# Acmece/rl-collision-avoidance

Hardware: AMD Instinct MI355X
Metric: agent-steps/s (N robots x 512-beam lidar) (higher is better)
Workload: dtype f32

## Files before the change

rl-collision-avoidance_amd/csrc/mrca_abi.hip:

```cpp
#include <hip/hip_runtime.h>
#include <string>
#include <chrono>

#include <algorithm>
#include <cmath>
#include <cstdarg>
#include <cstdio>
#include <cstdlib>
#include <cstring>
#include <memory>
#include <mutex>
#include <new>
#include <type_traits>
#include <utility>
#include <vector>

#include "../../include/mrca_env.h"
#include "mrca_host.h"
#include "mrca_hostutil.h"
#include "mrca_kernels.h"
#include "mrca_orca.h"
#include "mrca_dwa.h"
#include "mrca_pass_plan.h"
#include "mrca_render.h"
#include "mrca_rollout_store.h"

namespace {
thread_local char g_err[512] = "";
}

namespace mrca {
int set_error(int code, const char* fmt, ...) {
    va_list ap;
    va_start(ap, fmt);
    vsnprintf(g_err, sizeof(g_err), fmt, ap);
    va_end(ap);
    return code;
}
}

namespace {

using mrca::DeviceGuard;
using mrca::kAheadTicks;
#define fail(...) mrca::set_error(__VA_ARGS__)

#define HIP_TRY(expr)                                                                               \
    do {                                                                                            \
        hipError_t _e = (expr);                                                                     \
        if (_e != hipSuccess) return fail(MRCA_ERR_HIP, "%s failed: %s", #expr, hipGetErrorString(_e)); \
    } while (0)

constexpr size_t kAlign = 256;
size_t align_up(size_t v) { return (v + kAlign - 1) / kAlign * kAlign; }

struct Layout {
    size_t field_off[MRCA_F_COUNT];
    size_t field_bytes[MRCA_F_COUNT];
    size_t off_reset_mode, off_goal_mode, off_group_id, off_init_table, off_goal_table;
    size_t off_beam_cos, off_beam_sin, off_map, off_free_rect, off_cellfield, off_head, off_outline;
    size_t off_bw_ticket, off_bw_prov, off_bw_state, off_bw_chead, off_bw_cnext, off_bw_lstart, off_bw_lcount, off_bw_lsorted, off_bw_lblock, off_bw_lcursor;
    size_t off_status;
    int32_t bw_cmask, bw_lmask;
    size_t total;
};

int validate(const mrca_config* c) {
    if (!c) return fail(MRCA_ERR_INVALID, "config is NULL");
    if (c->abi_version != MRCA_ABI_VERSION)
        return fail(MRCA_ERR_INVALID, "abi_version %d != %d", c->abi_version, MRCA_ABI_VERSION);
    if (c->num_worlds < 1) return fail(MRCA_ERR_INVALID, "num_worlds must be >= 1");
    if (c->robots_per_world < 1) return fail(MRCA_ERR_INVALID, "robots_per_world must be >= 1");
    if (c->robots_per_world > 64 && c->auto_reset == MRCA_AUTO_GROUP)
        return fail(MRCA_ERR_UNSUPPORTED, "robots_per_world %d > 64 with group-synchronous episodes (auto_reset 2)",
                    c->robots_per_world);
    if (!(c->collision_raster >= 0.0f)) return fail(MRCA_ERR_INVALID, "collision_raster must be >= 0");
    if (c->collision_raster > 0.0f && (c->collision_raster < 0.1f || mrca::outline_span(1.0f / c->collision_raster) > mrca::kOutlineWin))
        return fail(MRCA_ERR_UNSUPPORTED, "collision_raster %.3f m: an outline is kept as an 8 x 8 bitmap of raster cells, which "
                    "holds cells of >= 0.1 m", (double)c->collision_raster);
    if (c->collision_raster > 0.0f && c->robots_per_world > 64)
        return fail(MRCA_ERR_UNSUPPORTED, "collision_raster with robots_per_world > 64");
    if ((int64_t)c->num_worlds * c->robots_per_world > (1 << 24))
        return fail(MRCA_ERR_UNSUPPORTED, "more than 2^24 robots in one environment");
    if (c->beams < 64 || c->beams > 1024 || c->beams % 64)
        return fail(MRCA_ERR_INVALID, "beams %d must be a multiple of 64 in [64,1024]", c->beams);
    if (c->frames < 1 || c->frames > 8) return fail(MRCA_ERR_INVALID, "frames %d out of [1,8]", c->frames);
    if (c->map_width < 1 || c->map_height < 1 || c->map_words_per_row < (c->map_width + 31) / 32)
        return fail(MRCA_ERR_INVALID, "bad map geometry %dx%d wpr %d", c->map_width, c->map_height,
                    c->map_words_per_row);
    if (c->map_width > 16384 || c->map_height > 16384)
        return fail(MRCA_ERR_UNSUPPORTED, "map %dx%d cells: at most 16384 per side", c->map_width, c->map_height);
    if (!(c->map_cell > 0.0f)) return fail(MRCA_ERR_INVALID, "map_cell must be > 0");
    if (!c->map_bits) return fail(MRCA_ERR_INVALID, "map_bits is NULL");
    if (c->auto_reset < 0 || c->auto_reset > 2) return fail(MRCA_ERR_INVALID, "auto_reset %d", c->auto_reset);
    const int R = c->robots_per_world;
    for (int i = 0; i < R; ++i) {
        if (c->reset_mode && (c->reset_mode[i] < 0 || c->reset_mode[i] > 2))
            return fail(MRCA_ERR_INVALID, "reset_mode[%d] = %d", i, c->reset_mode[i]);
        if (c->goal_mode && (c->goal_mode[i] < 0 || c->goal_mode[i] > 2))
            return fail(MRCA_ERR_INVALID, "goal_mode[%d] = %d", i, c->goal_mode[i]);
        if (c->group_id && (c->group_id[i] < 0 || c->group_id[i] > 15))
            return fail(MRCA_ERR_INVALID, "group_id[%d] = %d out of [0,15]", i, c->group_id[i]);
        if (c->reset_mode && c->reset_mode[i] == MRCA_RESET_TABLE && !c->init_table)
            return fail(MRCA_ERR_INVALID, "reset_mode[%d] is TABLE but init_table is NULL", i);
        if (c->goal_mode && c->goal_mode[i] == MRCA_RESET_TABLE && !c->goal_table)
            return fail(MRCA_ERR_INVALID, "goal_mode[%d] is TABLE but goal_table is NULL", i);
    }
    return MRCA_OK;
}

void make_layout(const mrca_config* c, Layout* L) {
    const size_t N = (size_t)c->num_worlds * c->robots_per_world;
    const size_t B = c->beams, F = c->frames, R = c->robots_per_world;
    size_t sz[MRCA_F_COUNT];
    sz[MRCA_F_POSE] = N * 3 * 4;
    sz[MRCA_F_SPEED] = N * 2 * 4;
    sz[MRCA_F_SPEED_GT] = N * 2 * 4;
    sz[MRCA_F_GOAL] = N * 2 * 4;
    sz[MRCA_F_INIT_POSE] = N * 3 * 4;
    sz[MRCA_F_SCAN] = N * B * 4;
    sz[MRCA_F_OBS] = N * F * B * 4;
    sz[MRCA_F_LOCAL_GOAL] = N * 2 * 4;
    sz[MRCA_F_REWARD] = N * 4;
    sz[MRCA_F_DONE] = N;
    sz[MRCA_F_RESULT] = N;
    sz[MRCA_F_FIRST_RESULT] = N;
    sz[MRCA_F_CRASHED] = N;
    sz[MRCA_F_LIVE] = N;
    sz[MRCA_F_FRESH] = N;
    sz[MRCA_F_T] = N * 4;
    sz[MRCA_F_EPISODE] = N * 4;
    sz[MRCA_F_PREV_DIST] = N * 4;
    sz[MRCA_F_SCAN_RING] = N * F * B * 4;
    sz[MRCA_F_RING_HEAD] = N;
    sz[MRCA_F_HIT_BITS] = N * F * (B / 64) * 8;
    size_t off = 0;
    for (int f = 0; f < MRCA_F_COUNT; ++f) {
        L->field_off[f] = off;
        L->field_bytes[f] = sz[f];
        off += align_up(sz[f]);
    }
    auto take = [&](size_t bytes) {
        size_t o = off;
        off += align_up(bytes);
        return o;
    };
    L->off_reset_mode = take(R * 4);
    L->off_goal_mode = take(R * 4);
    L->off_group_id = take(R * 4);
    L->off_init_table = take(R * 3 * 4);
    L->off_goal_table = take(R * 2 * 4);
    L->off_beam_cos = take(B * 4);
    L->off_beam_sin = take(B * 4);
    L->off_map = take((size_t)c->map_height * c->map_words_per_row * 4);
    L->off_free_rect = take((size_t)(c->map_width + 2 * mrca::kFieldPadX) * (c->map_height + 2 * mrca::kFieldPadY) *
                            4 * sizeof(uint16_t));
    L->off_cellfield = take((size_t)c->map_width * c->map_height);
    L->off_head = take(N * sizeof(float4));
    L->off_outline = take(c->collision_raster > 0.0f ? N * sizeof(mrca::OutlineBits) : 0);
    L->bw_cmask = L->bw_lmask = 0;
    if (c->robots_per_world > 64) {
        size_t mc = 1, ml = 1;
        while (mc < 4 * N) mc <<= 1;
        while (ml < 2 * N) ml <<= 1;
        L->bw_cmask = (int32_t)(mc - 1);
        L->bw_lmask = (int32_t)(ml - 1);
        L->off_bw_ticket = take(4);
        L->off_bw_prov = take(N * 2 * sizeof(float4));
        L->off_bw_state = take(N * 4);
        L->off_bw_chead = take(mc * 4);
        L->off_bw_cnext = take(2 * N * 4);
        L->off_bw_lstart = take((ml + 2) * 4);
        L->off_bw_lcount = take((ml + 1) * 4);
        L->off_bw_lsorted = take(N * 4);
// ... 196 lines not shown
    env->view.dev = env->view_dev.get();
    if ((e = hipDeviceSynchronize()) != hipSuccess) return e;
    return hipMemcpy(env->view_dev.get(), &env->view, sizeof(mrca::EnvView), hipMemcpyHostToDevice);
}

static int attach_arena(mrca_env* env, void* arena_dev, size_t arena_bytes) {
    const size_t total = env->layout.total;
    if (arena_dev) {
        if (arena_bytes < total) return fail(MRCA_ERR_NOMEM, "arena of %zu bytes < required %zu", arena_bytes, total);
        if (reinterpret_cast<uintptr_t>(arena_dev) % kAlign) return fail(MRCA_ERR_INVALID, "arena must be %zu-byte aligned", kAlign);
        env->arena = static_cast<char*>(arena_dev);
        return MRCA_OK;
    }
    const hipError_t e = device_alloc(&env->own_arena, total);
    if (e != hipSuccess) return fail(MRCA_ERR_NOMEM, "hipMalloc(%zu) failed: %s", total, hipGetErrorString(e));
    env->arena = env->own_arena.get();
    return MRCA_OK;
}

static int upload_tables(const mrca_config* cfg, const Layout& L, char* arena, int* free_rect_pitch, int* num_groups_out) {
    HIP_TRY(hipMemset(arena, 0, L.total));
    const int R = cfg->robots_per_world, B = cfg->beams;
    const size_t N = (size_t)cfg->num_worlds * R;
    std::vector<int32_t> reset_mode(R, MRCA_RESET_DISC), goal_mode(R, MRCA_RESET_DISC), group(R, 0);
    std::vector<float> init_tab(R * 3, 0.0f), goal_tab(R * 2, 0.0f);
    if (cfg->reset_mode) memcpy(reset_mode.data(), cfg->reset_mode, R * 4);
    if (cfg->goal_mode) memcpy(goal_mode.data(), cfg->goal_mode, R * 4);
    else if (cfg->reset_mode) goal_mode = reset_mode;
    if (cfg->group_id) memcpy(group.data(), cfg->group_id, R * 4);
    if (cfg->init_table) memcpy(init_tab.data(), cfg->init_table, R * 3 * 4);
    if (cfg->goal_table) memcpy(goal_tab.data(), cfg->goal_table, R * 2 * 4);
    int num_groups = 0;
    for (int i = 0; i < R; ++i) num_groups = group[i] + 1 > num_groups ? group[i] + 1 : num_groups;
    *num_groups_out = num_groups;
    std::vector<float> bcos(B), bsin(B);
    for (int i = 0; i < B; ++i) {
        const double b = -M_PI / 2.0 + (double)i * (M_PI / (double)(B - 1));
        bcos[i] = (float)std::cos(b);
        bsin[i] = (float)std::sin(b);
    }
    HIP_TRY(hipMemcpy(arena + L.off_reset_mode, reset_mode.data(), R * 4, hipMemcpyHostToDevice));
    HIP_TRY(hipMemcpy(arena + L.off_goal_mode, goal_mode.data(), R * 4, hipMemcpyHostToDevice));
    HIP_TRY(hipMemcpy(arena + L.off_group_id, group.data(), R * 4, hipMemcpyHostToDevice));
    HIP_TRY(hipMemcpy(arena + L.off_init_table, init_tab.data(), R * 3 * 4, hipMemcpyHostToDevice));
    HIP_TRY(hipMemcpy(arena + L.off_goal_table, goal_tab.data(), R * 2 * 4, hipMemcpyHostToDevice));
    {
        std::vector<float> pose0((size_t)N * 3);
        for (size_t n = 0; n < N; ++n)
            for (int k = 0; k < 3; ++k) pose0[n * 3 + k] = init_tab[(n % (size_t)R) * 3 + k];
        HIP_TRY(hipMemcpy(arena + L.field_off[MRCA_F_POSE], pose0.data(), pose0.size() * 4, hipMemcpyHostToDevice));
    }
    HIP_TRY(hipMemcpy(arena + L.off_beam_cos, bcos.data(), B * 4, hipMemcpyHostToDevice));
    HIP_TRY(hipMemcpy(arena + L.off_beam_sin, bsin.data(), B * 4, hipMemcpyHostToDevice));
    HIP_TRY(hipMemcpy(arena + L.off_map, cfg->map_bits, (size_t)cfg->map_height * cfg->map_words_per_row * 4,
                      hipMemcpyHostToDevice));
    {
        const std::shared_ptr<const HostField> hf = host_field(cfg, false);
        *free_rect_pitch = hf->pitch;
        HIP_TRY(hipMemcpy(arena + L.off_free_rect, hf->entries.data(), hf->entries.size() * sizeof(uint16_t),
                          hipMemcpyHostToDevice));
    }
    {
        std::vector<uint8_t> cf;
        mrca::build_cell_field(cfg->map_bits, cfg->map_width, cfg->map_height, cfg->map_words_per_row, &cf);
        HIP_TRY(hipMemcpy(arena + L.off_cellfield, cf.data(), cf.size(), hipMemcpyHostToDevice));
    }
    if (R > 64)
        HIP_TRY(hipMemset(arena + L.off_bw_chead, 0xFF, ((size_t)L.bw_cmask + 1) * 4));
    HIP_TRY(hipMemset(arena + L.field_off[MRCA_F_LIVE], 1, N));
    {
        std::vector<int32_t> ones(N, 1);
        HIP_TRY(hipMemcpy(arena + L.field_off[MRCA_F_T], ones.data(), N * 4, hipMemcpyHostToDevice));
    }
    return MRCA_OK;
}

static bool field_octants(const mrca_config* c) {
    if (const char* v = std::getenv("MRCA_FIELD_OCTANTS")) return std::atoi(v) != 0;
    const size_t bytes = (size_t)(c->map_width + 2 * mrca::kFieldPadX) * (c->map_height + 2 * mrca::kFieldPadY) * 8 * sizeof(uint16_t);
    return c->lazy_obs != 0 && bytes <= ((size_t)4 << 20);
}

static int upload_octants(const mrca_config* cfg, mrca_env* env) {
    const std::shared_ptr<const HostField> hf = host_field(cfg, true);
    const size_t bytes = hf->octants.size() * sizeof(uint16_t);
    HIP_TRY(device_alloc(&env->octant_rect, bytes));
    HIP_TRY(hipMemcpy(env->octant_rect.get(), hf->octants.data(), bytes, hipMemcpyHostToDevice));
    env->view.march_rect = env->octant_rect.get();
    env->view.march_shift = 4;
    env->view.march_major = 8;
    return MRCA_OK;
}

static mrca::EnvView make_view(const mrca_config* cfg, const Layout& L, char* a, int free_rect_pitch, int num_groups) {
    const int R = cfg->robots_per_world, B = cfg->beams;
    const size_t N = (size_t)cfg->num_worlds * R;
    mrca::EnvView v = mrca::EnvView();
    v.N = (int32_t)N;
    v.R = R;
    v.W = cfg->num_worlds;
    v.B = B;
    v.F = cfg->frames;
    v.pose = reinterpret_cast<float*>(a + L.field_off[MRCA_F_POSE]);
    v.speed = reinterpret_cast<float*>(a + L.field_off[MRCA_F_SPEED]);
    v.speed_gt = reinterpret_cast<float*>(a + L.field_off[MRCA_F_SPEED_GT]);
    v.goal = reinterpret_cast<float*>(a + L.field_off[MRCA_F_GOAL]);
    v.init_pose = reinterpret_cast<float*>(a + L.field_off[MRCA_F_INIT_POSE]);
    v.scan = reinterpret_cast<float*>(a + L.field_off[MRCA_F_SCAN]);
    v.obs = reinterpret_cast<float*>(a + L.field_off[MRCA_F_OBS]);
    v.scan_ring = reinterpret_cast<float*>(a + L.field_off[MRCA_F_SCAN_RING]);
    v.ring_head = reinterpret_cast<uint8_t*>(a + L.field_off[MRCA_F_RING_HEAD]);
    v.hit_bits = reinterpret_cast<unsigned long long*>(a + L.field_off[MRCA_F_HIT_BITS]);
    v.local_goal = reinterpret_cast<float*>(a + L.field_off[MRCA_F_LOCAL_GOAL]);
    v.reward = reinterpret_cast<float*>(a + L.field_off[MRCA_F_REWARD]);
    v.prev_dist = reinterpret_cast<float*>(a + L.field_off[MRCA_F_PREV_DIST]);
    v.done = reinterpret_cast<uint8_t*>(a + L.field_off[MRCA_F_DONE]);
    v.result = reinterpret_cast<uint8_t*>(a + L.field_off[MRCA_F_RESULT]);
    v.first_result = reinterpret_cast<uint8_t*>(a + L.field_off[MRCA_F_FIRST_RESULT]);
    v.crashed = reinterpret_cast<uint8_t*>(a + L.field_off[MRCA_F_CRASHED]);
    v.live = reinterpret_cast<uint8_t*>(a + L.field_off[MRCA_F_LIVE]);
    v.fresh = reinterpret_cast<uint8_t*>(a + L.field_off[MRCA_F_FRESH]);
    v.t = reinterpret_cast<int32_t*>(a + L.field_off[MRCA_F_T]);
    v.episode = reinterpret_cast<int32_t*>(a + L.field_off[MRCA_F_EPISODE]);
    v.reset_mode = reinterpret_cast<const int32_t*>(a + L.off_reset_mode);
    v.goal_mode = reinterpret_cast<const int32_t*>(a + L.off_goal_mode);
    v.group_id = reinterpret_cast<const int32_t*>(a + L.off_group_id);
    v.init_table = reinterpret_cast<const float*>(a + L.off_init_table);
    v.goal_table = reinterpret_cast<const float*>(a + L.off_goal_table);
    v.beam_cos = reinterpret_cast<const float*>(a + L.off_beam_cos);
    v.beam_sin = reinterpret_cast<const float*>(a + L.off_beam_sin);
    v.beam_step = mrca::kPi / (float)(B - 1);
    v.beam_inv_step = (float)(B - 1) / mrca::kPi;
    v.map_bits = reinterpret_cast<const uint32_t*>(a + L.off_map);
    v.free_rect = reinterpret_cast<const uint16_t*>(a + L.off_free_rect);
    v.free_rect_pitch = free_rect_pitch;
    v.march_rect = v.free_rect;
    v.march_shift = 3;
    v.march_major = 0;
    v.cellfield = reinterpret_cast<const uint8_t*>(a + L.off_cellfield);
    v.head = reinterpret_cast<float4*>(a + L.off_head);
    v.outline = cfg->collision_raster > 0.0f ? reinterpret_cast<mrca::OutlineBits*>(a + L.off_outline) : nullptr;
    v.big = R > 64 ? 1 : 0;
    if (v.big) {
        v.bw_ticket = reinterpret_cast<uint32_t*>(a + L.off_bw_ticket);
        v.bw_prov = reinterpret_cast<float4*>(a + L.off_bw_prov);
        v.bw_state = reinterpret_cast<int32_t*>(a + L.off_bw_state);
        v.bw_chead = reinterpret_cast<int32_t*>(a + L.off_bw_chead);
        v.bw_cnext = reinterpret_cast<int32_t*>(a + L.off_bw_cnext);
        v.bw_lstart = reinterpret_cast<int32_t*>(a + L.off_bw_lstart);
        v.bw_lcount = reinterpret_cast<int32_t*>(a + L.off_bw_lcount);
        v.bw_lsorted = reinterpret_cast<int32_t*>(a + L.off_bw_lsorted);
        v.bw_lblock = reinterpret_cast<int32_t*>(a + L.off_bw_lblock);
        v.bw_lcursor = reinterpret_cast<int32_t*>(a + L.off_bw_lcursor);
        v.bw_cmask = L.bw_cmask;
        v.bw_lmask = L.bw_lmask;
    }
    v.status = reinterpret_cast<uint32_t*>(a + L.off_status);
    v.ray_first = 0;
    v.ray_count = (int32_t)N;
    v.world_first = 0;
    v.world_count = cfg->num_worlds;
    v.g.x0 = cfg->map_x0;
    v.g.y0 = cfg->map_y0;
    v.g.cell = cfg->map_cell;
    v.g.inv_cell = 1.0f / cfg->map_cell;
    v.g.width = cfg->map_width;
// ... 953 lines not shown
```

rl-collision-avoidance_amd/csrc/mrca_device.h:

```cpp
#pragma once
#include <stdint.h>
#include <math.h>
#include <string.h>

#if defined(__HIPCC__)
#define MRCA_HD __host__ __device__ __forceinline__
#else
#define MRCA_HD inline
#endif

namespace mrca {

constexpr float kDt = 0.1f;
constexpr float kRangeMax = 6.0f;
constexpr float kHalfLen = 0.22f;
constexpr float kHalfWid = 0.19f;
constexpr float kGoalRadius = 0.5f;
constexpr float kRArrive = 15.0f;
constexpr float kRCrash = -15.0f;
constexpr float kKProgress = 2.5f;
constexpr float kKOmega = -0.1f;
constexpr float kPi = 3.14159265358979323846f;
constexpr float kTwoPi = 6.28318530717958647692f;
constexpr int kMaxTriesPose = 64;
// ... 71 lines not shown
    MRCA_HD bool operator()(int ix, int iy) const {
        if (ix < 0 || iy < 0 || ix >= width || iy >= height) return false;
        return in_map(ix, iy);
    }
    MRCA_HD bool in_map(int ix, int iy) const {
        return (bits[(uint32_t)(iy * wpr + (ix >> 5))] >> (ix & 31)) & 1u;
    }
};

template <class Occ>
MRCA_HD float grid_march(const Occ& occ, const GridGeom& g, float ox, float oy, float dx, float dy, float tmax) {
    const float fx = (ox - g.x0) * g.inv_cell;
    const float fy = (oy - g.y0) * g.inv_cell;
    int ix = (int)floorf(fx);
    int iy = (int)floorf(fy);
    const float tmax_c = tmax * g.inv_cell;
    if (occ(ix, iy)) return 0.0f;
    if (!(tmax_c > 0.0f)) return tmax;
    const bool xnz = dx != 0.0f, ynz = dy != 0.0f;
    const float inv_dx = xnz ? rcp_exact(dx) : kInf;
    const float inv_dy = ynz ? rcp_exact(dy) : kInf;
    const int sx = dx > 0.0f ? 1 : -1;
    const int sy = dy > 0.0f ? 1 : -1;
    int bx = dx > 0.0f ? ix + 1 : ix;
    int by = dy > 0.0f ? iy + 1 : iy;
    float tx = xnz ? ((float)bx - fx) * inv_dx : kInf;
    float ty = ynz ? ((float)by - fy) * inv_dy : kInf;
    for (int guard = 0; guard < kMaxMarchSteps; ++guard) {
        float t;
        if (tx < ty) {
            t = tx;
            ix += sx;
            bx += sx;
            tx = ((float)bx - fx) * inv_dx;
        } else {
            t = ty;
            iy += sy;
            by += sy;
            ty = ynz ? ((float)by - fy) * inv_dy : kInf;
        }
        if (t >= tmax_c) return tmax;
        if (occ(ix, iy)) return t * g.cell;
    }
    return tmax;
}

constexpr int kFieldMaxExtent = 254;
constexpr uint32_t kCellOccupied = 0xFFFFu;

constexpr int kFieldPadX = 2, kFieldPadY = 1;
MRCA_HD int imin(int a, int b) { return a < b ? a : b; }
MRCA_HD int imax(int a, int b) { return a > b ? a : b; }

MRCA_HD int med3_i32(int a, int b, int c) {
#if defined(__HIP_DEVICE_COMPILE__)
    int r;
    asm("v_med3_i32 %0, %1, %2, %3" : "=v"(r) : "v"(a), "v"(b), "v"(c));
    return r;
#else
    const int lo = imin(a, imin(b, c)), hi = imax(a, imax(b, c));
    return a + b + c - lo - hi;
#endif
}
MRCA_HD int mad24(int a, int b, int c) {
#if defined(__HIP_DEVICE_COMPILE__)
    int r;
    asm("v_mad_i32_i24 %0, %1, %2, %3" : "=v"(r) : "v"(a), "v"(b), "v"(c));
    return r;
#else
    return a * b + c;
#endif
}
template <int LO>
MRCA_HD int clamp_from(int x, int hi) {
#if defined(__HIP_DEVICE_COMPILE__)
    int r;
    asm("v_med3_i32 %0, %1, %2, %3" : "=v"(r) : "v"(x), "n"(LO), "s"(hi));
    return r;
#else
    return imin(imax(x, LO), hi);
#endif
}

struct FreeRectField {
    const uint16_t* d;
    int32_t w, h, pitch;
    uint32_t shift = 3, major = 0;
    MRCA_HD uint32_t cell_offset(int ix, int iy) const {
        const int x = clamp_from<-kFieldPadX>(ix, w + kFieldPadX - 1);
        const int y = clamp_from<-kFieldPadY>(iy, h + kFieldPadY - 1);
#if defined(__HIP_DEVICE_COMPILE__)
        const int idx = __mul24(y, pitch) + x;
#else
        const int idx = y * pitch + x;
#endif
        return (uint32_t)(idx + (kFieldPadY * pitch + kFieldPadX)) << shift;
    }
    MRCA_HD uint32_t entry_bytes(float dx, float dy) const {
        return (dx > 0.0f ? 2u : 0u) + (dy > 0.0f ? 4u : 0u) + (__builtin_fabsf(dx) >= __builtin_fabsf(dy) ? major : 0u);
    }
    MRCA_HD uint32_t operator()(int ix, int iy, uint32_t qbytes) const {
        return *reinterpret_cast<const uint16_t*>(reinterpret_cast<const char*>(d) + (cell_offset(ix, iy) + qbytes));
    }
    MRCA_HD void cell(int ix, int iy, uint32_t* lo, uint32_t* hi) const {
        const uint32_t* p = reinterpret_cast<const uint32_t*>(reinterpret_cast<const char*>(d) + cell_offset(ix, iy));
        *lo = p[0];
        *hi = p[1];
    }
};

struct MarchOrigin {
    float fx, fy;
    int32_t ix0, iy0;
    uint32_t v_lo, v_hi;
};
template <class Field>
MRCA_HD MarchOrigin march_origin(const Field& field, const GridGeom& g, float ox, float oy) {
    MarchOrigin o;
    o.fx = (ox - g.x0) * g.inv_cell;
    o.fy = (oy - g.y0) * g.inv_cell;
    o.ix0 = (int)floorf(o.fx);
    o.iy0 = (int)floorf(o.fy);
    field.cell(o.ix0, o.iy0, &o.v_lo, &o.v_hi);
    return o;
}

MRCA_HD float at_or_before(float t, bool inclusive) {
    uint32_t u;
    __builtin_memcpy(&u, &t, 4);
    u = (u & 0x7FFFFFFFu) + (inclusive ? 1u : 0u);
    float r;
    __builtin_memcpy(&r, &u, 4);
    return r;
}

MRCA_HD int lane_counter(int x) {
#if defined(__HIP_DEVICE_COMPILE__)
    asm("" : "+v"(x));
#endif
    return x;
}

template <class Field>
MRCA_HD float grid_march_skip(const Field& field, const GridGeom& g, const MarchOrigin& org, float dx, float dy,
                              float tmax) {
    const float fx = org.fx, fy = org.fy;
    const int ix0 = org.ix0, iy0 = org.iy0;
    const float tmax_c = tmax * g.inv_cell;
    const bool xnz = dx != 0.0f, ynz = dy != 0.0f;
    const bool xpos = dx > 0.0f, ypos = dy > 0.0f;
    const uint32_t qbytes = field.entry_bytes(dx, dy);
    const uint32_t vq = ypos ? org.v_hi : org.v_lo;
    uint32_t v = xpos ? vq >> 16 : vq & 0xFFFFu;
    if (v == kCellOccupied) return 0.0f;
    if (!(tmax_c > 0.0f)) return tmax;
    const float rdx = rcp_exact(dx), rdy = rcp_exact(dy);
    const float inv_dx = xnz ? rdx : kInf;
    const float inv_dy = ynz ? rdy : kInf;
    const int sx = xpos ? 1 : -1, sy = ypos ? 1 : -1;
    const int ux = xpos ? 1 : 0, uy = ypos ? 1 : 0;
    const int limx = xpos ? 0x3FFFFFFF : -0x3FFFFFFF, limy = ypos ? 0x3FFFFFFF : -0x3FFFFFFF;
    const bool bothnz = xnz & ynz;
    int bx = ix0 + ux;
    int by = iy0 + uy;
    float out = tmax;
    int left = lane_counter(kMaxMarchSteps);
    do {
        const int ex = (int)(v & 255u), ey = (int)((v >> 8) & 255u);
        const int Bx = mad24(ex, sx, bx);
        const int By = mad24(ey, sy, by);
        const float rawx = ((float)Bx - fx) * inv_dx;
        const float rawy = ((float)By - fy) * inv_dy;
        const float tBx = xnz ? rawx : kInf;
        const float tBy = ynz ? rawy : kInf;
        const bool xe = tBx < tBy;
        const float t = xe ? tBx : tBy;
        if (t >= tmax_c) {
            left = 0;
        } else {
            const float fS = xe ? fy : fx;
            const float invS = xe ? inv_dy : inv_dx;
            const int sS = xe ? sy : sx;
            const int bS0 = xe ? by : bx;
            const float pT = fS + (xe ? dy : dx) * t;
            const int b = med3_i32((int)floorf(pT) + (xe ? uy : ux), bS0, xe ? limy : limx);
            const int bprev = b - sS;
            const float tp = ((float)bprev - fS) * invS;
            const float tc = ((float)b - fS) * invS;
            const float tle = at_or_before(t, xe);
            const bool cons_p = tp < tle;
            const bool cons_c = tc < tle;
            int bS = cons_c ? b + sS : b;
            bS = ((b != bS0) & !cons_p) ? bprev : bS;
            bS = bothnz ? bS : bS0;
            bx = xe ? Bx + sx : bS;
            by = xe ? bS : By + sy;
            v = field(bx - ux, by - uy, qbytes);
            const bool hit = v == kCellOccupied;
            out = hit ? t * g.cell : out;
            left = hit ? 0 : left - 1;
        }
        left = lane_counter(left);
    } while (left > 0);
    return out;
}

template <class Field>
MRCA_HD float grid_march_skip(const Field& field, const GridGeom& g, float ox, float oy, float dx, float dy,
                              float tmax) {
    return grid_march_skip(field, g, march_origin(field, g, ox, oy), dx, dy, tmax);
}

template <int K, class Field>
MRCA_HD void grid_march_skip_n(const Field& field, const GridGeom& g, const MarchOrigin& org, const float (&dx)[K],
                               const float (&dy)[K], float tmax, float (&out)[K]) {
    const float fx = org.fx, fy = org.fy;
    const float tmax_c = tmax * g.inv_cell;
    if ((org.v_lo & 0xFFFFu) == kCellOccupied) {
#pragma unroll
        for (int k = 0; k < K; ++k) out[k] = 0.0f;
        return;
    }
    if (!(tmax_c > 0.0f)) {
#pragma unroll
        for (int k = 0; k < K; ++k) out[k] = tmax;
        return;
    }
    float inv_dx[K], inv_dy[K], t[K];
    int bx[K], by[K];
    uint32_t v[K], qb[K];
    bool act[K], hit[K];
#pragma unroll
    for (int k = 0; k < K; ++k) {
        inv_dx[k] = dx[k] != 0.0f ? rcp_exact(dx[k]) : kInf;
        inv_dy[k] = dy[k] != 0.0f ? rcp_exact(dy[k]) : kInf;
        bx[k] = org.ix0 + (dx[k] > 0.0f ? 1 : 0);
        by[k] = org.iy0 + (dy[k] > 0.0f ? 1 : 0);
        qb[k] = field.entry_bytes(dx[k], dy[k]);
        const uint32_t vq = dy[k] > 0.0f ? org.v_hi : org.v_lo;
        v[k] = dx[k] > 0.0f ? vq >> 16 : vq & 0xFFFFu;
        t[k] = 0.0f;
        act[k] = true;
        hit[k] = false;
    }
    int guard = kMaxMarchSteps;
    bool any = true;
    while (any) {
        int cx[K], cy[K], nbx[K], nby[K];
        float tn[K];
        bool go[K];
#pragma unroll
        for (int k = 0; k < K; ++k) {
            const bool xnz = dx[k] != 0.0f, ynz = dy[k] != 0.0f;
            const bool xpos = dx[k] > 0.0f, ypos = dy[k] > 0.0f;
            const int sx = xpos ? 1 : -1, sy = ypos ? 1 : -1;
            const int ux = xpos ? 1 : 0, uy = ypos ? 1 : 0;
            const int limx = xpos ? 0x3FFFFFFF : -0x3FFFFFFF, limy = ypos ? 0x3FFFFFFF : -0x3FFFFFFF;
            const int ex = (int)(v[k] & 255u), ey = (int)((v[k] >> 8) & 255u);
            const int Bx = mad24(ex, sx, bx[k]);
            const int By = mad24(ey, sy, by[k]);
            const float rawx = ((float)Bx - fx) * inv_dx[k];
            const float rawy = ((float)By - fy) * inv_dy[k];
            const float tBx = xnz ? rawx : kInf;
            const float tBy = ynz ? rawy : kInf;
            const bool xe = tBx < tBy;
            const float tt = xe ? tBx : tBy;
            const float fS = xe ? fy : fx;
            const float invS = xe ? inv_dy[k] : inv_dx[k];
            const int sS = xe ? sy : sx;
            const int bS0 = xe ? by[k] : bx[k];
            int bS = bS0;
            if (xnz & ynz) {
                const float pT = fS + (xe ? dy[k] : dx[k]) * tt;
                const int b = med3_i32((int)floorf(pT) + (xe ? uy : ux), bS0, xe ? limy : limx);
                const int bprev = b - sS;
                const float tp = ((float)bprev - fS) * invS;
                const float tc = ((float)b - fS) * invS;
                const bool cons_p = (tp < tt) | ((tp == tt) & xe);
                const bool cons_c = (tc < tt) | ((tc == tt) & xe);
                bS = cons_c ? b + sS : b;
                bS = ((b != bS0) & !cons_p) ? bprev : bS;
            }
            go[k] = act[k] && !(tt >= tmax_c);
            tn[k] = tt;
            nbx[k] = go[k] ? (xe ? Bx + sx : bS) : bx[k];
            nby[k] = go[k] ? (xe ? bS : By + sy) : by[k];
            cx[k] = nbx[k] - ux;
// ... 598 lines not shown
```

rl-collision-avoidance_amd/csrc/mrca_host.h:

```cpp
#pragma once
#include <stdint.h>

#include <algorithm>
#include <thread>
#include <vector>

#include "mrca_device.h"

namespace mrca {

inline void build_free_rect_field(const uint32_t* bits, int width, int height, int wpr, std::vector<uint16_t>* out,
                                  int* pitch_out) {
    const size_t sw = (size_t)width + 1;
    std::vector<int32_t> sat(sw * ((size_t)height + 1), 0);
    auto occupied = [&](int x, int y) -> int { return (bits[(size_t)y * wpr + (x >> 5)] >> (x & 31)) & 1u; };
    for (int y = 0; y < height; ++y)
        for (int x = 0; x < width; ++x)
            sat[(size_t)(y + 1) * sw + x + 1] =
                occupied(x, y) + sat[(size_t)y * sw + x + 1] + sat[(size_t)(y + 1) * sw + x] - sat[(size_t)y * sw + x];
    auto count = [&](int x0, int y0, int x1, int y1) -> int {
        if (x0 > x1) std::swap(x0, x1);
        if (y0 > y1) std::swap(y0, y1);
        x0 = std::max(x0, 0); y0 = std::max(y0, 0); x1 = std::min(x1, width - 1); y1 = std::min(y1, height - 1);
        if (x0 > x1 || y0 > y1) return 0;
        return sat[(size_t)(y1 + 1) * sw + x1 + 1] - sat[(size_t)y0 * sw + x1 + 1] - sat[(size_t)(y1 + 1) * sw + x0] +
               sat[(size_t)y0 * sw + x0];
    };
    const int pitch = width + 2 * kFieldPadX;
    out->assign((size_t)pitch * (height + 2 * kFieldPadY) * 4, 0);
    uint16_t* field = out->data();
    auto rows = [&](int y_begin, int y_end) {
        const int M = kFieldMaxExtent;
        for (int y = y_begin; y < y_end; ++y)
            for (int x = 0; x < width; ++x) {
                uint16_t* e = field + ((size_t)(y + kFieldPadY) * pitch + x + kFieldPadX) * 4;
                if (occupied(x, y)) {
                    e[0] = e[1] = e[2] = e[3] = (uint16_t)kCellOccupied;
                    continue;
                }
                for (int q = 0; q < 4; ++q) {
                    const int sx = (q & 1) ? 1 : -1, sy = (q & 2) ? 1 : -1;
                    int ex = 0, ey = 0;
                    for (bool grew = true; grew;) {
                        grew = false;
                        if (ex < M && count(x + sx * (ex + 1), y, x + sx * (ex + 1), y + sy * ey) == 0) { ++ex; grew = true; }
                        if (ey < M && count(x, y + sy * (ey + 1), x + sx * ex, y + sy * (ey + 1)) == 0) { ++ey; grew = true; }
                    }
                    e[q] = (uint16_t)(ex | (ey << 8));
                }
            }
    };
    const int nthreads = std::max(1, std::min({(int)std::thread::hardware_concurrency(), 16, height / 64}));
    std::vector<std::thread> pool;
    for (int t = 1; t < nthreads; ++t)
        pool.emplace_back(rows, (int)((int64_t)height * t / nthreads), (int)((int64_t)height * (t + 1) / nthreads));
    rows(0, height / nthreads);
    for (std::thread& th : pool) th.join();
    *pitch_out = pitch;
}

inline void build_octant_rect_field(const uint32_t* bits, int width, int height, int wpr, std::vector<uint16_t>* out,
                                    int* pitch_out, int RX = 2, int RY = 1, int MAXE = kFieldMaxExtent) {
    const size_t sw = (size_t)width + 1;
    std::vector<int32_t> sat(sw * ((size_t)height + 1), 0);
    auto occupied = [&](int x, int y) -> int { return (bits[(size_t)y * wpr + (x >> 5)] >> (x & 31)) & 1u; };
    for (int y = 0; y < height; ++y)
        for (int x = 0; x < width; ++x)
            sat[(size_t)(y + 1) * sw + x + 1] =
                occupied(x, y) + sat[(size_t)y * sw + x + 1] + sat[(size_t)(y + 1) * sw + x] - sat[(size_t)y * sw + x];
    auto count = [&](int x0, int y0, int x1, int y1) -> int {
        if (x0 > x1) std::swap(x0, x1);
        if (y0 > y1) std::swap(y0, y1);
        x0 = std::max(x0, 0); y0 = std::max(y0, 0); x1 = std::min(x1, width - 1); y1 = std::min(y1, height - 1);
        if (x0 > x1 || y0 > y1) return 0;
        return sat[(size_t)(y1 + 1) * sw + x1 + 1] - sat[(size_t)y0 * sw + x1 + 1] - sat[(size_t)(y1 + 1) * sw + x0] +
               sat[(size_t)y0 * sw + x0];
    };
    const int pitch = width + 2 * kFieldPadX;
    out->assign((size_t)pitch * (height + 2 * kFieldPadY) * 8, 0);
    uint16_t* field = out->data();
    auto rows = [&](int y_begin, int y_end) {
        const int M = std::min(MAXE, kFieldMaxExtent);
        for (int y = y_begin; y < y_end; ++y)
            for (int x = 0; x < width; ++x) {
                uint16_t* e = field + ((size_t)(y + kFieldPadY) * pitch + x + kFieldPadX) * 8;
                if (occupied(x, y)) {
                    for (int k = 0; k < 8; ++k) e[k] = (uint16_t)kCellOccupied;
                    continue;
                }
                for (int k = 0; k < 8; ++k) {
                    const int q = k & 3;
                    const int sx = (q & 1) ? 1 : -1, sy = (q & 2) ? 1 : -1;
// ... 51 lines not shown
```

rl-collision-avoidance_amd/csrc/mrca_raycast_body.h:

```cpp
#pragma once
#include "mrca_kernels.h"

namespace mrca {

namespace {

#if !defined(MRCA_RSTAMP)
#define MRCA_RSTAMP(k) do { } while (0)
#endif

typedef __attribute__((address_space(1))) uint8_t GlobalByte;
struct RayTick {
    int j, T;
    const uint8_t* fresh0;
    long long stride;
    const uint8_t* fresh_env;
    const uint8_t* head_in;
    uint8_t* head_out;
};

__device__ __forceinline__ void mask_or(unsigned long long* p, unsigned long long v) {
    (void)__hip_atomic_fetch_or(p, v, __ATOMIC_RELAXED, __HIP_MEMORY_SCOPE_WORKGROUP);
}

__device__ __forceinline__ int block_to_robot(int b, int N) {
    const uint32_t ub = (uint32_t)b, un = (uint32_t)N;
    if (un & 7u) return b;
    return (int)((ub & 7u) * (un >> 3) + (ub >> 3));
}

template <int K, bool BIG, bool SEQ, int RKW, bool VIEWS, bool TICKS = false>
__device__ __forceinline__ void raycast_body(int only_fresh, int ray_first, int ray_count, int R_, const float* __restrict__ pose_p,
                                             const float4* __restrict__ head_p, const float* __restrict__ bcos_p,
                                             const float* __restrict__ bsin_p, uint8_t* ring_head_p, const EnvView& e, int views,
                                             const RayTick& mt = RayTick{}) {
    extern __shared__ __attribute__((aligned(16))) uint32_t lds[];
    MRCA_RSTAMP(0);
    const int n = ray_first + block_to_robot(blockIdx.x, ray_count);
    const int tid = threadIdx.x;
    if (only_fresh && e.fresh[n] == 0) return;

    float4* nb = reinterpret_cast<float4*>(lds);
    int2* nbi = reinterpret_cast<int2*>(nb + kWave);
    int* nb_count = reinterpret_cast<int*>(nbi + kWave);
    unsigned long long* nbmask = reinterpret_cast<unsigned long long*>(nb_count + 4);
    int* nb_more = nb_count + 1;
    constexpr bool raster = RKW > 0 && !BIG;
    int4* nbo = reinterpret_cast<int4*>(nbmask + e.B);

    const int T = e.B / K;
    const bool extra = (int)blockDim.x > T;
    const int prep_base = extra ? T : 0;
    const bool is_prep = tid >= prep_base && tid < prep_base + kWave;
    const bool marches = tid < T;
    const int world = BIG ? n / R_ : (R_ == 1 ? n : (int)__umulhi((uint32_t)n, e.r_magic));
    const int local = n - world * R_;
    int lane_zero = 0;
    if constexpr (!BIG) asm volatile("v_mov_b32 %0, 0" : "=v"(lane_zero));
    const int nv = n + lane_zero;
    const float x = pose_p[nv * 3 + 0], y = pose_p[nv * 3 + 1];
    const float4 hd = head_p[nv];
    const float s = hd.x, c = hd.y;
    const int pl = tid - prep_base;
    const bool cand = !BIG && is_prep && (pl < R_) && (pl != local);
    const int jn = world * R_ + (cand ? pl : local);
    float xj = 0.0f, yj = 0.0f;
    float4 hj = make_float4(0.0f, 0.0f, 0.0f, 0.0f);
    int4 oj = make_int4(0, 0, 0, 0);
    if (!BIG && is_prep) {
        xj = pose_p[jn * 3 + 0];
        yj = pose_p[jn * 3 + 1];
        if constexpr (raster) oj = reinterpret_cast<const int4*>(e.outline)[jn];
        else hj = head_p[jn];
    }
    float bc[K], bs[K];
#pragma unroll
    for (int k = 0; k < K; ++k) {
        const int b = (marches ? tid : 0) + k * T;
        bc[k] = bcos_p[b];
        bs[k] = bsin_p[b];
    }
    uint8_t fresh_byte;
    int ring_slot;
    if constexpr (TICKS) {
        const int lt = tid & (kWave - 1);
        const int t = lt < mt.T ? lt : 0;
        const bool own = mt.fresh_env != nullptr && t == mt.T - 1;
        const unsigned long long fa = own ? (unsigned long long)mt.fresh_env : (unsigned long long)mt.fresh0 + (long long)t * mt.stride;
        fresh_byte = *reinterpret_cast<const GlobalByte*>(fa + (unsigned long long)n);
        ring_slot = mt.head_in[nv];
    } else {
        fresh_byte = e.fresh[n];
        ring_slot = ring_head_p[n];
    }
    int big_off = 0;
    auto big_chunk = [&]() {
        const int icx = hash_cell_coord(x, kLidarCell), icy = hash_cell_coord(y, kLidarCell);
        for (int b = pl; b < e.B; b += kWave) nbmask[b] = 0ull;
        int cell_start = 0, cell_count = 0;
        if (pl < 9) {
            const uint32_t h = hash_cell(icx + pl % 3 - 1, icy + pl / 3 - 1, world) & (uint32_t)e.bw_lmask;
            cell_start = e.bw_lstart[h];
            cell_count = e.bw_lstart[h + 1] - cell_start;
        }
        int cell_end = cell_count;
#pragma unroll
        for (int d = 1; d < 16; d <<= 1) {
            const int up = __shfl_up(cell_end, d, kWave);
            if (pl >= d) cell_end += up;
        }
        const int total = __shfl(cell_end, 8, kWave);
        int cnt = 0;
        while (big_off < total) {
            const int entry = big_off + pl;
            int q = 0;
#pragma unroll
            for (int t = 0; t < 8; ++t) q += __shfl(cell_end, t, kWave) <= entry ? 1 : 0;
            const bool valid = entry < total;
            q = valid ? q : 0;
            const int qx = icx + q % 3 - 1, qy = icy + q / 3 - 1;
            const int q_end = __shfl(cell_end, q, kWave), q_count = __shfl(cell_count, q, kWave);
            const int idx = __shfl(cell_start, q, kWave) + (entry - (q_end - q_count));
            const int j = valid ? e.bw_lsorted[idx] : -1;
            bool keep = false;
            float cxj = 0.0f, cyj = 0.0f;
            float4 chj = make_float4(0.0f, 0.0f, 0.0f, 0.0f);
            int lo = 0, hi = -1;
            if (j >= 0 && j != n && j / R_ == world) {
                cxj = pose_p[j * 3 + 0];
                cyj = pose_p[j * 3 + 1];
                if (hash_cell_coord(cxj, kLidarCell) == qx && hash_cell_coord(cyj, kLidarCell) == qy) {
                    const float ddx = cxj - x, ddy = cyj - y;
                    if (ddx * ddx + ddy * ddy <= kLidarReach2) {
                        beam_interval(ddx * c + ddy * s, ddy * c - ddx * s, e.B, e.beam_step, e.beam_inv_step, e.lidar_radius,
                                      e.lidar_near, &lo, &hi);
                        keep = lo <= hi;
                        if (keep) chj = head_p[j];
                    }
                }
            }
            const unsigned long long m = __ballot(keep);
            const int add = __popcll(m);
            if (cnt + add > kWave) break;
            if (keep) {
                const int idx2 = cnt + __popcll(m & ((1ull << pl) - 1ull));
                float olx, oly;
                ray_box_origin(x, y, cxj, cyj, chj.x, chj.y, &olx, &oly);
                nb[idx2] = make_float4(olx, oly, chj.x, chj.y);
                nbi[idx2] = make_int2(lo, hi);
            }
            cnt += add;
            big_off += kWave;
        }
        if (pl == 0) {
            *nb_count = MRCA_DBG(e, 1) ? 0 : cnt;
            *nb_more = big_off < total ? 1 : 0;
        }
        for (int k = 0; k < cnt; ++k) {
            const int2 iv = nbi[k];
            for (int b = iv.x + pl; b <= iv.y; b += kWave) mask_or(&nbmask[b], 1ull << k);
        }
    };
    MRCA_RSTAMP(1);
    if (is_prep) {
      if constexpr (BIG) {
        big_chunk();
      } else {
        for (int b = pl; b < e.B; b += kWave) nbmask[b] = 0ull;
        const float ddx = xj - x, ddy = yj - y;
        bool keep = cand && (ddx * ddx + ddy * ddy <= e.lidar_reach2);
        int lo = 0, hi = -1;
        if (keep) {
            beam_interval(ddx * c + ddy * s, ddy * c - ddx * s, e.B, e.beam_step, e.beam_inv_step, e.lidar_radius, e.lidar_near,
                          &lo, &hi);
            keep = lo <= hi;
        }
        const unsigned long long m = __ballot(keep);
        if (keep) {
            const int idx = __popcll(m & ((1ull << pl) - 1ull));
            if constexpr (raster) {
                nbo[idx] = oj;
            } else {
                float olx, oly;
                ray_box_origin(x, y, xj, yj, hj.x, hj.y, &olx, &oly);
                nb[idx] = make_float4(olx, oly, hj.x, hj.y);
            }
            nbi[idx] = make_int2(lo, hi);
        }
        const int cnt0 = MRCA_DBG(e, 1) ? 0 : __popcll(m);
        if (pl == 0) *nb_count = cnt0;
        for (int k = 0; k < cnt0; ++k) {
            const int2 iv = nbi[k];
            for (int b = iv.x + pl; b <= iv.y; b += kWave) mask_or(&nbmask[b], 1ull << k);
        }
      }
    }
    MRCA_RSTAMP(2);
    float dx[K], dy[K], rng[K];
    bool from_robot[K];
#pragma unroll
    for (int k = 0; k < K; ++k) {
        dx[k] = c * bc[k] - s * bs[k];
        dy[k] = s * bc[k] + c * bs[k];
        rng[k] = kRangeMax;
        from_robot[k] = false;
    }
// ... 27 lines not shown
    MRCA_RSTAMP(4);
    if constexpr (!BIG) {
        if (!marches) return;
    }
    for (;;) {
        const int cnt = *nb_count;
        const int more = BIG ? *nb_more : 0;
        if (marches) {
#pragma unroll
            for (int k = 0; k < K; ++k) {
                const int b = tid + k * T;
                float r = rng[k];
                unsigned long long m = cnt > 0 ? nbmask[b] : 0ull;
                if constexpr (raster) {
                    if (m) {
                        const float fxr = x * e.raster_inv, fyr = y * e.raster_inv;
                        const int ixr = (int)floorf(fxr), iyr = (int)floorf(fyr);
                        const float tmax_c = kRangeMax * e.raster_inv;
                        const float inv_dx = dx[k] != 0.0f ? rcp_exact(dx[k]) : kInf;
                        const float inv_dy = dy[k] != 0.0f ? rcp_exact(dy[k]) : kInf;
                        const float fxe = dx[k] != 0.0f ? fxr : -kInf, fye = dy[k] != 0.0f ? fyr : -kInf;
                        const bool xpos = dx[k] > 0.0f, ypos = dy[k] > 0.0f;
                        do {
                            const int q = __ffsll((long long)m) - 1;
                            m &= m - 1;
                            const int4 oq = nbo[q];
                            const OutlineBits ob{oq.x, oq.y, (uint32_t)oq.z, (uint32_t)oq.w};
                            const float tc = RKW == 4 ? ray_outline_entry4(fxe, fye, ixr, iyr, xpos, ypos, inv_dx, inv_dy, ob)
                                                      : ray_outline_entry<RKW>(fxr, fyr, ixr, iyr, dx[k], dy[k], inv_dx, inv_dy, ob);
                            const float t = tc < tmax_c ? tc * e.raster_res : kInf;
                            from_robot[k] = from_robot[k] || t < r;
                            r = t < r ? t : r;
                        } while (m);
                    }
                } else {
                    while (m) {
                        const int q = __ffsll((long long)m) - 1;
                        m &= m - 1;
                        const float4 nbq = nb[q];
                        const float t = ray_box_local(nbq.x, nbq.y, dx[k], dy[k], nbq.z, nbq.w);
                        from_robot[k] = from_robot[k] || t < r;
                        r = t < r ? t : r;
                    }
                }
                rng[k] = r;
            }
        }
        if (!more) break;
        __syncthreads();
        if (is_prep) big_chunk();
        __syncthreads();
    }
    if (!marches) return;
    MRCA_RSTAMP(5);
    {
        const uint32_t row = (uint32_t)n * (uint32_t)e.F;
        float* ring_row = e.scan_ring + (size_t)row * (uint32_t)e.B;
        const int words = e.B >> 6;
        unsigned long long* hit_row = e.hit_bits + (size_t)row * (uint32_t)words;
        int new_slot;
        bool fresh;
        uint32_t stores = 0u;
        int head_after = 0;
        if constexpr (TICKS) {
            const uint32_t fresh_bits = (uint32_t)__ballot(fresh_byte != 0 && (tid & (kWave - 1)) < mt.T);
            const RingStores rs = ring_rule(e.F, mt.T, ring_slot, fresh_bits, mt.j);
            stores = (uint32_t)__builtin_amdgcn_readfirstlane((int)rs.stores);
            head_after = rs.head;
            fresh = ((fresh_bits >> mt.j) & 1u) != 0u;
            new_slot = __ffs((int)stores) - 1;
        } else {
            new_slot = ring_slot + 1 == e.F ? 0 : ring_slot + 1;
            fresh = __builtin_amdgcn_readfirstlane((int)fresh_byte) != 0;
        }
#pragma unroll
        for (int k = 0; k < K; ++k) {
            const int b = tid + k * T;
            const float r = rng[k] < kRangeMax ? rng[k] : kRangeMax;
            const unsigned long long hm = __ballot(from_robot[k] && rng[k] < kRangeMax);
            const bool word_lane = (tid & (kWave - 1)) == 0;
            if (fresh) {
                for (int f = 0; f < e.F; ++f) {
                    if (TICKS && !((stores >> f) & 1u)) continue;
                    __builtin_nontemporal_store(r, &ring_row[f * e.B + b]);
                    if (word_lane) hit_row[f * words + (b >> 6)] = hm;
                }
            } else if (!TICKS || stores) {
                __builtin_nontemporal_store(r, &ring_row[new_slot * e.B + b]);
                if (word_lane) hit_row[new_slot * words + (b >> 6)] = hm;
            }
            if (VIEWS && views) {
                const float nr = norm_obs(r);
                if (views & 1) __builtin_nontemporal_store(r, &e.scan[(size_t)n * (uint32_t)e.B + b]);
                if (views & 2) {
                    float* dst = e.obs + (size_t)row * (uint32_t)e.B + b;
                    if (fresh) {
                        for (int f = 0; f < e.F; ++f) __builtin_nontemporal_store(nr, &dst[f * e.B]);
                    } else {
                        int slot = new_slot;
                        for (int f = 0; f < e.F - 1; ++f) {
                            slot = slot + 1 == e.F ? 0 : slot + 1;
                            __builtin_nontemporal_store(norm_obs(fabsf(ring_row[slot * e.B + b])), &dst[f * e.B]);
                        }
                        __builtin_nontemporal_store(nr, &dst[(e.F - 1) * e.B]);
                    }
                }
            }
        }
        if constexpr (TICKS) {
            if (tid == 0 && mt.j == mt.T - 1) mt.head_out[n] = (uint8_t)head_after;
        } else {
            if (tid == 0 && !fresh) ring_head_p[n] = (uint8_t)new_slot;
        }
    }
    if (tid == 0 && (!TICKS || mt.j == mt.T - 1)) {
        const float gx = e.goal[n * 2 + 0] - x, gy = e.goal[n * 2 + 1] - y;
        e.local_goal[n * 2 + 0] = gx * c + gy * s;
        e.local_goal[n * 2 + 1] = gy * c - gx * s;
    }
    MRCA_RSTAMP(6);
}

}

}
```

Before: 267.5 million.

## Use 32-bit global address-space offsets and wave-uniform control in grid march

Adds global_load/store helpers that cast pointers to the global address space and index with 32-bit byte offsets. This lets the compiler emit global (not flat) memory instructions with saddr+voffset addressing, which cuts 64-bit address arithmetic in the raycast and field lookups. The grid-march loop is also restructured to branch on a wave-wide ballot instead of per-lane divergence, with the hit result computed after the loop. New checks ensure field arrays fit 32-bit offsets, so octant fields on very large maps are rejected.

```diff
diff --git a/rl-collision-avoidance_amd/csrc/mrca_abi.hip b/rl-collision-avoidance_amd/csrc/mrca_abi.hip
--- a/rl-collision-avoidance_amd/csrc/mrca_abi.hip
+++ b/rl-collision-avoidance_amd/csrc/mrca_abi.hip
@@ -88,8 +88,9 @@
     if (c->map_width < 1 || c->map_height < 1 || c->map_words_per_row < (c->map_width + 31) / 32)
         return fail(MRCA_ERR_INVALID, "bad map geometry %dx%d wpr %d", c->map_width, c->map_height,
                     c->map_words_per_row);
-    if (c->map_width > 16384 || c->map_height > 16384)
-        return fail(MRCA_ERR_UNSUPPORTED, "map %dx%d cells: at most 16384 per side", c->map_width, c->map_height);
+    static_assert(mrca::field_fits_offsets(mrca::kMaxMapSide, mrca::kMaxMapSide, 4), "the quadrant array of the largest map");
+    if (c->map_width > mrca::kMaxMapSide || c->map_height > mrca::kMaxMapSide)
+        return fail(MRCA_ERR_UNSUPPORTED, "map %dx%d cells: at most %d per side", c->map_width, c->map_height, mrca::kMaxMapSide);
     if (!(c->map_cell > 0.0f)) return fail(MRCA_ERR_INVALID, "map_cell must be > 0");
     if (!c->map_bits) return fail(MRCA_ERR_INVALID, "map_bits is NULL");
     if (c->auto_reset < 0 || c->auto_reset > 2) return fail(MRCA_ERR_INVALID, "auto_reset %d", c->auto_reset);
@@ -452,6 +453,9 @@
 }
 
 static int upload_octants(const mrca_config* cfg, mrca_env* env) {
+    if (!mrca::field_fits_offsets(cfg->map_width, cfg->map_height, 8))
+        return fail(MRCA_ERR_UNSUPPORTED, "map %dx%d cells: the octant free-rectangle array passes 4 GiB (MRCA_FIELD_OCTANTS=0 "
+                    "marches over the quadrant array)", cfg->map_width, cfg->map_height);
     const std::shared_ptr<const HostField> hf = host_field(cfg, true);
     const size_t bytes = hf->octants.size() * sizeof(uint16_t);
     HIP_TRY(device_alloc(&env->octant_rect, bytes));
diff --git a/rl-collision-avoidance_amd/csrc/mrca_device.h b/rl-collision-avoidance_amd/csrc/mrca_device.h
--- a/rl-collision-avoidance_amd/csrc/mrca_device.h
+++ b/rl-collision-avoidance_amd/csrc/mrca_device.h
@@ -177,6 +177,28 @@
 #endif
 }
 
+#if defined(__HIP_DEVICE_COMPILE__)
+#define MRCA_GLOBAL __attribute__((address_space(1)))
+#else
+#define MRCA_GLOBAL
+#endif
+template <class T>
+MRCA_HD T global_load(const void* base, uint32_t byte_off) {
+    return *reinterpret_cast<const MRCA_GLOBAL T*>((const MRCA_GLOBAL char*)base + byte_off);
+}
+template <class T>
+MRCA_HD void global_store(void* base, uint32_t byte_off, T v) {
+    *reinterpret_cast<MRCA_GLOBAL T*>((MRCA_GLOBAL char*)base + byte_off) = v;
+}
+template <class T>
+MRCA_HD void global_store_nt(void* base, uint32_t byte_off, T v) {
+#if defined(__HIP_DEVICE_COMPILE__)
+    __builtin_nontemporal_store(v, reinterpret_cast<MRCA_GLOBAL T*>((MRCA_GLOBAL char*)base + byte_off));
+#else
+    global_store<T>(base, byte_off, v);
+#endif
+}
+
 struct FreeRectField {
     const uint16_t* d;
     int32_t w, h, pitch;
@@ -195,12 +217,12 @@
         return (dx > 0.0f ? 2u : 0u) + (dy > 0.0f ? 4u : 0u) + (__builtin_fabsf(dx) >= __builtin_fabsf(dy) ? major : 0u);
     }
     MRCA_HD uint32_t operator()(int ix, int iy, uint32_t qbytes) const {
-        return *reinterpret_cast<const uint16_t*>(reinterpret_cast<const char*>(d) + (cell_offset(ix, iy) + qbytes));
+        return global_load<uint16_t>(d, cell_offset(ix, iy) + qbytes);
     }
     MRCA_HD void cell(int ix, int iy, uint32_t* lo, uint32_t* hi) const {
-        const uint32_t* p = reinterpret_cast<const uint32_t*>(reinterpret_cast<const char*>(d) + cell_offset(ix, iy));
-        *lo = p[0];
-        *hi = p[1];
+        const uint32_t off = cell_offset(ix, iy);
+        *lo = global_load<uint32_t>(d, off);
+        *hi = global_load<uint32_t>(d, off + 4u);
     }
 };
 
@@ -236,14 +258,45 @@
     return x;
 }
 
+MRCA_HD float lane_value(float x) {
+#if defined(__HIP_DEVICE_COMPILE__)
+    asm("" : "+v"(x));
+#endif
+    return x;
+}
+MRCA_HD bool wave_any(bool c) {
+#if defined(__HIP_DEVICE_COMPILE__)
+    return __builtin_amdgcn_ballot_w64(c) != 0ull;
+#else
+    return c;
+#endif
+}
+
+MRCA_HD float idle_axis_origin(float f, bool travels) {
+#if defined(__HIP_DEVICE_COMPILE__)
+    return travels ? f : -kInf;
+#else
+    (void)travels;
+    return f;
+#endif
+}
+MRCA_HD float idle_axis_time(float raw, bool travels) {
+#if defined(__HIP_DEVICE_COMPILE__)
+    (void)travels;
+    return raw;
+#else
+    return travels ? raw : kInf;
+#endif
+}
+
 template <class Field>
 MRCA_HD float grid_march_skip(const Field& field, const GridGeom& g, const MarchOrigin& org, float dx, float dy,
                               float tmax) {
-    const float fx = org.fx, fy = org.fy;
     const int ix0 = org.ix0, iy0 = org.iy0;
     const float tmax_c = tmax * g.inv_cell;
     const bool xnz = dx != 0.0f, ynz = dy != 0.0f;
     const bool xpos = dx > 0.0f, ypos = dy > 0.0f;
+    const float fx = idle_axis_origin(org.fx, xnz), fy = idle_axis_origin(org.fy, ynz);
     const uint32_t qbytes = field.entry_bytes(dx, dy);
     const uint32_t vq = ypos ? org.v_hi : org.v_lo;
     uint32_t v = xpos ? vq >> 16 : vq & 0xFFFFu;
@@ -254,31 +307,27 @@
     const float inv_dy = ynz ? rdy : kInf;
     const int sx = xpos ? 1 : -1, sy = ypos ? 1 : -1;
     const int ux = xpos ? 1 : 0, uy = ypos ? 1 : 0;
-    const int limx = xpos ? 0x3FFFFFFF : -0x3FFFFFFF, limy = ypos ? 0x3FFFFFFF : -0x3FFFFFFF;
     const bool bothnz = xnz & ynz;
     int bx = ix0 + ux;
     int by = iy0 + uy;
-    float out = tmax;
     int left = lane_counter(kMaxMarchSteps);
+    float t;
     do {
         const int ex = (int)(v & 255u), ey = (int)((v >> 8) & 255u);
         const int Bx = mad24(ex, sx, bx);
         const int By = mad24(ey, sy, by);
-        const float rawx = ((float)Bx - fx) * inv_dx;
-        const float rawy = ((float)By - fy) * inv_dy;
-        const float tBx = xnz ? rawx : kInf;
-        const float tBy = ynz ? rawy : kInf;
+        const float tBx = idle_axis_time(((float)Bx - fx) * inv_dx, xnz);
+        const float tBy = idle_axis_time(((float)By - fy) * inv_dy, ynz);
         const bool xe = tBx < tBy;
-        const float t = xe ? tBx : tBy;
-        if (t >= tmax_c) {
-            left = 0;
-        } else {
+        t = xe ? tBx : tBy;
+        const bool go = !(t >= tmax_c);
+        if (wave_any(go)) {
             const float fS = xe ? fy : fx;
             const float invS = xe ? inv_dy : inv_dx;
             const int sS = xe ? sy : sx;
             const int bS0 = xe ? by : bx;
             const float pT = fS + (xe ? dy : dx) * t;
-            const int b = med3_i32((int)floorf(pT) + (xe ? uy : ux), bS0, xe ? limy : limx);
+            const int b = med3_i32((int)floorf(pT) + (xe ? uy : ux), bS0, (int)((uint32_t)sS << 30));
             const int bprev = b - sS;
             const float tp = ((float)bprev - fS) * invS;
             const float tc = ((float)b - fS) * invS;
@@ -291,13 +340,13 @@
             bx = xe ? Bx + sx : bS;
             by = xe ? bS : By + sy;
             v = field(bx - ux, by - uy, qbytes);
-            const bool hit = v == kCellOccupied;
-            out = hit ? t * g.cell : out;
-            left = hit ? 0 : left - 1;
         }
-        left = lane_counter(left);
+        v = go ? v : kCellOccupied;
+        left = lane_counter(v == kCellOccupied ? 0 : left - 1);
     } while (left > 0);
-    return out;
+    t = lane_value(t);
+    v = (uint32_t)lane_counter((int)v);
+    return (!(t >= tmax_c) & (v == kCellOccupied)) ? t * g.cell : tmax;
 }
 
 template <class Field>
diff --git a/rl-collision-avoidance_amd/csrc/mrca_host.h b/rl-collision-avoidance_amd/csrc/mrca_host.h
--- a/rl-collision-avoidance_amd/csrc/mrca_host.h
+++ b/rl-collision-avoidance_amd/csrc/mrca_host.h
@@ -8,6 +8,12 @@
 #include "mrca_device.h"
 
 namespace mrca {
+
+constexpr int kMaxMapSide = 16384;
+constexpr bool field_fits_offsets(int width, int height, int entries) {
+    return (uint64_t)(width + 2 * kFieldPadX) * (uint64_t)(height + 2 * kFieldPadY) * (uint64_t)entries * sizeof(uint16_t) <=
+           0xFFFFFFFFull;
+}
 
 inline void build_free_rect_field(const uint32_t* bits, int width, int height, int wpr, std::vector<uint16_t>* out,
                                   int* pitch_out) {
diff --git a/rl-collision-avoidance_amd/csrc/mrca_raycast_body.h b/rl-collision-avoidance_amd/csrc/mrca_raycast_body.h
--- a/rl-collision-avoidance_amd/csrc/mrca_raycast_body.h
+++ b/rl-collision-avoidance_amd/csrc/mrca_raycast_body.h
@@ -70,7 +70,7 @@
     if (!BIG && is_prep) {
         xj = pose_p[jn * 3 + 0];
         yj = pose_p[jn * 3 + 1];
-        if constexpr (raster) oj = reinterpret_cast<const int4*>(e.outline)[jn];
+        if constexpr (raster) oj = global_load<int4>(e.outline, (uint32_t)jn * 16u);
         else hj = head_p[jn];
     }
     float bc[K], bs[K];
@@ -100,8 +100,8 @@
         int cell_start = 0, cell_count = 0;
         if (pl < 9) {
             const uint32_t h = hash_cell(icx + pl % 3 - 1, icy + pl / 3 - 1, world) & (uint32_t)e.bw_lmask;
-            cell_start = e.bw_lstart[h];
-            cell_count = e.bw_lstart[h + 1] - cell_start;
+            cell_start = global_load<int>(e.bw_lstart, h * 4u);
+            cell_count = global_load<int>(e.bw_lstart, h * 4u + 4u) - cell_start;
         }
         int cell_end = cell_count;
 #pragma unroll
@@ -121,7 +121,7 @@
             const int qx = icx + q % 3 - 1, qy = icy + q / 3 - 1;
             const int q_end = __shfl(cell_end, q, kWave), q_count = __shfl(cell_count, q, kWave);
             const int idx = __shfl(cell_start, q, kWave) + (entry - (q_end - q_count));
-            const int j = valid ? e.bw_lsorted[idx] : -1;
+            const int j = valid ? global_load<int>(e.bw_lsorted, (uint32_t)idx * 4u) : -1;
             bool keep = false;
             float cxj = 0.0f, cyj = 0.0f;
             float4 chj = make_float4(0.0f, 0.0f, 0.0f, 0.0f);
@@ -315,41 +315,42 @@
             if (fresh) {
                 for (int f = 0; f < e.F; ++f) {
                     if (TICKS && !((stores >> f) & 1u)) continue;
-                    __builtin_nontemporal_store(r, &ring_row[f * e.B + b]);
-                    if (word_lane) hit_row[f * words + (b >> 6)] = hm;
+                    global_store_nt(ring_row, (uint32_t)(f * e.B + b) * 4u, r);
+                    if (word_lane) global_store(hit_row, (uint32_t)(f * words + (b >> 6)) * 8u, hm);
                 }
             } else if (!TICKS || stores) {
-                __builtin_nontemporal_store(r, &ring_row[new_slot * e.B + b]);
-                if (word_lane) hit_row[new_slot * words + (b >> 6)] = hm;
+                global_store_nt(ring_row, (uint32_t)(new_slot * e.B + b) * 4u, r);
+                if (word_lane) global_store(hit_row, (uint32_t)(new_slot * words + (b >> 6)) * 8u, hm);
             }
             if (VIEWS && views) {
                 const float nr = norm_obs(r);
-                if (views & 1) __builtin_nontemporal_store(r, &e.scan[(size_t)n * (uint32_t)e.B + b]);
+                if (views & 1) global_store_nt(e.scan + (size_t)n * (uint32_t)e.B, (uint32_t)b * 4u, r);
                 if (views & 2) {
-                    float* dst = e.obs + (size_t)row * (uint32_t)e.B + b;
+                    float* dst = e.obs + (size_t)row * (uint32_t)e.B;
                     if (fresh) {
-                        for (int f = 0; f < e.F; ++f) __builtin_nontemporal_store(nr, &dst[f * e.B]);
+                        for (int f = 0; f < e.F; ++f) global_store_nt(dst, (uint32_t)(f * e.B + b) * 4u, nr);
                     } else {
                         int slot = new_slot;
                         for (int f = 0; f < e.F - 1; ++f) {
                             slot = slot + 1 == e.F ? 0 : slot + 1;
-                            __builtin_nontemporal_store(norm_obs(fabsf(ring_row[slot * e.B + b])), &dst[f * e.B]);
+                            const float older = global_load<float>(ring_row, (uint32_t)(slot * e.B + b) * 4u);
+                            global_store_nt(dst, (uint32_t)(f * e.B + b) * 4u, norm_obs(fabsf(older)));
                         }
-                        __builtin_nontemporal_store(nr, &dst[(e.F - 1) * e.B]);
+                        global_store_nt(dst, (uint32_t)((e.F - 1) * e.B + b) * 4u, nr);
                     }
                 }
             }
         }
         if constexpr (TICKS) {
-            if (tid == 0 && mt.j == mt.T - 1) mt.head_out[n] = (uint8_t)head_after;
+            if (tid == 0 && mt.j == mt.T - 1) global_store(mt.head_out, (uint32_t)n, (uint8_t)head_after);
         } else {
-            if (tid == 0 && !fresh) ring_head_p[n] = (uint8_t)new_slot;
+            if (tid == 0 && !fresh) global_store(ring_head_p, (uint32_t)n, (uint8_t)new_slot);
         }
     }
     if (tid == 0 && (!TICKS || mt.j == mt.T - 1)) {
-        const float gx = e.goal[n * 2 + 0] - x, gy = e.goal[n * 2 + 1] - y;
-        e.local_goal[n * 2 + 0] = gx * c + gy * s;
-        e.local_goal[n * 2 + 1] = gy * c - gx * s;
+        const float gx = global_load<float>(e.goal, (uint32_t)n * 8u) - x, gy = global_load<float>(e.goal, (uint32_t)n * 8u + 4u) - y;
+        global_store(e.local_goal, (uint32_t)n * 8u, gx * c + gy * s);
+        global_store(e.local_goal, (uint32_t)n * 8u + 4u, gy * c - gx * s);
     }
     MRCA_RSTAMP(6);
 }
```

Measured after the change: 275.2 million, median of 6. 2.9% higher.
